# JJanai/back2future

Hardware: AMD Instinct MI355X
Metric: frame-triplets/sec at 3x1024x1920 (higher is better)
Workload: dtype f32; 1 GPU; BASELINE.json configs[4] per-GPU share: batch=16 synthetic 3x1024x1920 triplets per GPU, random-init pwc.lua weights (Ours-Hard shape), outputs flow + occ + est[3]; batch_per_gpu=16, global_batch=16, height=1024, width=1920, parallelism=dp1: independent triplets per rank, one RCCL weight broadcast at init, hip_graph=True

## Files before the change

### back2future_amd/csrc/b2f_api.hip

```cpp
#include "b2f_ctx.h"

#include <cctype>
#include <cmath>
#include <cstdio>
#include <cstdlib>

using namespace b2f;

static thread_local std::string g_err;
namespace b2f {
int api_fail(const std::string &m)
{
    g_err = m;
    return 1;
}
const std::string &api_error() { return g_err; }

ConvSeg cp8_seg(const float *ptr, int C, size_t hw)
{
    ConvSeg sgm;
    sgm.ptr = ptr;
    sgm.img_stride = (long)(hw * (size_t)((C + 7) / 8 * 8));
    sgm.chunk_stride = (long)(hw * 8);
    sgm.pix_stride = 8;
    sgm.nchunks = 0;
    return sgm;
}
}
static int fail(const std::string &m) { return api_fail(m); }

namespace {

int prof_id(b2f_ctx *c, const char *name)
{
    for (size_t i = 0; i < c->prof_names.size(); ++i)
        if (c->prof_names[i] == name) return (int)i;
    c->prof_names.push_back(name);
    c->prof_ms.push_back(0.0);
    c->prof_n.push_back(0);
    return (int)c->prof_names.size() - 1;
}

hipEvent_t get_event(b2f_ctx *c)
{
    if (!c->ev_pool.empty()) {
        hipEvent_t e = c->ev_pool.back();
        c->ev_pool.pop_back();
        return e;
    }
    hipEvent_t e = nullptr;
    (void)hipEventCreate(&e);
    return e;
}

struct Scope {
    b2f_ctx *c;
    hipStream_t s;
    ProfEvent pe;
    bool on;
    Scope(b2f_ctx *c_, hipStream_t s_, const char *name, bool capturing) : c(c_), s(s_), on(c_->profile && !capturing)
    {
        if (on) {
            pe.name = prof_id(c, name);
            pe.a = get_event(c);
            pe.b = get_event(c);
            (void)hipEventRecord(pe.a, s);
        }
    }
    ~Scope()
    {
        if (on) {
            (void)hipEventRecord(pe.b, s);
            c->prof_pending.push_back(pe);
        }
    }
};

int prof_collect(b2f_ctx *c)
{
    for (ProfEvent &pe : c->prof_pending) {
        HIPCHK(hipEventSynchronize(pe.b));
        float ms = 0.f;
        HIPCHK(hipEventElapsedTime(&ms, pe.a, pe.b));
        c->prof_ms[pe.name] += ms;
        c->prof_n[pe.name] += 1;
        c->ev_pool.push_back(pe.a);
        c->ev_pool.push_back(pe.b);
    }
    c->prof_pending.clear();
    return 0;
}

int find_conv(const b2f_ctx *c, int kind, int level, int idx);

bool use_wino()
{
    static const bool on = !(getenv("B2F_WINO") && atoi(getenv("B2F_WINO")) == 0);
    return on;
}

struct KernelRow {
    const char *tag[2];
    const char *cls[2];
    void (*tiles)(int co, int *nt, int *nblk);
    size_t (*w_floats)(int chunks, int co, int nt, int nblk);
    bool bias;
    void (*pack)(const float *w, const float *b, int co, int ci, const int *cin_map, int chunks, int nt, int nblk, float *wpk, float *bpk);
    hipError_t (*launch)(const ConvLaunch &, hipStream_t);
};
#define TL [](int co, int *nt, int *nblk)
#define WF [](int chunks, int co, int nt, int nblk) -> size_t
#define PK [](const float *w, const float *b, int co, int ci, const int *m, int chunks, int nt, int nblk, float *wpk, float *bpk)
const KernelRow kKernels[K_COUNT] = {
    {{"D1", "D2"}, {"conv3x3_s1_nt%d", "conv3x3_s2_nt%d"}, conv_choose_tiles, WF { return conv_wpk_floats(chunks, nt, nblk); }, true,
     PK { conv_pack_weights(w, b, co, ci, m, chunks, nt, nblk, wpk, bpk); }, launch_conv3x3},
    {{"N2", "N2"}, {"conv3x3_narrow2", "conv3x3_narrow2"}, TL { *nt = 1; *nblk = 1; }, WF { return narrow2_wpk_floats(chunks); }, true,
     PK { narrow2_pack_weights(w, b, ci, m, chunks, wpk, bpk); }, launch_conv_narrow2},
    {{"W2", "W2"}, {"conv3x3_wino_nt%d", "conv3x3_wino_nt%d"}, wino_choose_tiles, WF { return wino_wpk_floats(chunks, nt, nblk); }, true,
     PK { wino_pack_weights(w, b, co, ci, m, chunks, nt, nblk, wpk, bpk); }, launch_conv3x3_wino},
    {{"C16", "C16"}, {"conv3x3_c16_%d", "conv3x3_c16_%d"}, TL { *nt = 1; *nblk = 1; }, WF { return c16_wpk_floats(); }, true,
     PK { c16_pack_weights(w, b, ci, m, wpk, bpk); }, launch_conv3x3_c16},
    {{"S16", "S16"}, {"conv3x3_s2x16_%d", "conv3x3_s2x16_%d"}, TL { *nt = 1; *nblk = 1; }, WF { return c16s2_wpk_floats(); }, true,
     PK { c16s2_pack_weights(w, b, ci, m, wpk, bpk); }, launch_conv3x3_c16s2},
    {{"W4", "W4"}, {"conv3x3_wino4_nt%d", "conv3x3_wino4_nt%d"}, TL { *nt = 2; *nblk = wino4_nblk(co); }, WF { return wino4_wpk_floats(chunks, nblk); }, true,
     PK { wino4_pack_weights(w, b, co, ci, m, chunks, nblk, wpk, bpk); }, launch_conv3x3_wino4},
    {{"E1", "E2"}, {"conv3x3_s1_bf16_%d", "conv3x3_s2_bf16_%d"}, TL { *nt = 2; *nblk = convb_nblk(co); }, WF { return convb_wpk_floats(chunks, co); }, true,
     PK { convb_pack_weights(w, b, co, ci, m, chunks, wpk, bpk); }, launch_conv3x3_bf6},
    {{"L2", "L2"}, {"conv3x3_s2b_%d", "conv3x3_s2b_%d"}, TL { *nt = 1; *nblk = s2b_ntiles(co); }, WF { return s2b_wpk_floats(chunks, co); }, true,
     PK { s2b_pack_weights(w, b, co, ci, m, chunks, wpk, bpk); }, launch_conv3x3_s2b},
    {{"V1", "V1"}, {"conv3x3_w1b_%d", "conv3x3_w1b_%d"}, TL { *nt = 2; *nblk = w1b_nblk(co); }, WF { return w1b_wpk_floats(chunks, co); }, true,
     PK { w1b_pack_weights(w, b, co, ci, m, chunks, wpk, bpk); },
     [](const ConvLaunch &L, hipStream_t s) {
         const hipError_t e = launch_conv3x3_w1b(L, s);
         return e == hipSuccess && L.w1b_nblk < w1b_nblk(L.cout) ? launch_conv3x3_wino4_rem(L, s) : e;
     }},
    {{"W6", "W6"}, {"conv3x3_wino6_nt%d", "conv3x3_wino6_nt%d"}, TL { *nt = 2; *nblk = wino6_nblk(co); }, WF { return wino6_wpk_floats(chunks, co); }, true,
     PK { wino6_pack_weights(w, b, co, ci, m, chunks, wpk, bpk); }, launch_conv3x3_wino6},
#if B2F_EXPERIMENTS
    {{nullptr, nullptr}, {nullptr, nullptr}, TL { *nt = 2; *nblk = wino4_nblk(co); }, WF { return wino4s_wpk_floats(chunks, nblk); }, false,
     PK { wino4s_pack_weights(w, co, ci, m, chunks, nblk, wpk); }, nullptr},
    {{nullptr, nullptr}, {nullptr, nullptr}, TL { *nt = 2; *nblk = wino4_nblk(co); }, WF { return wino2s_wpk_floats(chunks, nblk); }, false,
     PK { wino2s_pack_weights(w, co, ci, m, chunks, nblk, wpk); }, nullptr},
#endif
};
#undef TL
#undef WF
#undef PK

ConvKernel base_kernel(int ci, int co, bool stride1, bool two_segments)
{
    static const int min4 = getenv("B2F_WINO4_MIN_COUT") ? atoi(getenv("B2F_WINO4_MIN_COUT")) : 32;
    static const int min2 = getenv("B2F_WINO_MIN_COUT") ? atoi(getenv("B2F_WINO_MIN_COUT")) : 16;
    if (!use_wino()) return K_DIRECT;
    if (ci == 16 && co == (stride1 ? 16 : 32)) return stride1 ? K_C16 : K_C16S2;
    if (!stride1) return K_DIRECT;
    if (co == 2) return two_segments ? K_DIRECT : K_NARROW2;
    if (co < min2) return K_DIRECT;
    return (min4 > 0 && co >= min4 && co % 4 == 0) ? K_WINO4 : K_WINO2;
}

bool packs(const PackedConv &p, ConvKernel k, bool stride1, const KernelOpts &o)
{
    const bool w4 = p.base == K_WINO4;
    switch (k) {
    case K_BF6: return (p.base == K_DIRECT || (w4 && o.bf16_conv >= 2)) && (p.cout & 3) == 0;
    case K_S2B: return p.base == K_DIRECT && !stride1 && (p.cout & 31) == 0 && p.cout <= 256;
    case K_WINO2: return w4 || p.base == K_WINO2;
    case K_W1B: return w4 && o.wino1d;
    case K_WINO6: return w4 && o.wino6;
#if B2F_EXPERIMENTS
    case K_WINO4S: return w4 && (o.wino4_split || o.wino4_hybrid);
    case K_WINO2S: return w4 && o.wino2_split;
#endif
    default: return k == p.base;
    }
}

void place_packings(PackedConv &p, bool stride1, const KernelOpts &o, size_t *total)
{
    for (int k = 0; k < K_COUNT; ++k) {
        if (!packs(p, (ConvKernel)k, stride1, o)) continue;
        PackedConv::Packing &q = p.pk[k];
        kKernels[k].tiles(p.cout, &q.nt, &q.nblk);
        q.w_off = *total = (*total + 3) & ~(size_t)3;
        q.b_off = *total += kKernels[k].w_floats(p.nchunks(), p.cout, q.nt, q.nblk);
        if (kKernels[k].bias) *total += (size_t)q.nblk * q.nt * 32;
    }
}

void fill_packings(const PackedConv &p, const float *w, const float *b, int ci, const int *cin_map, float *host)
{
    for (int k = 0; k < K_COUNT; ++k)
        if (p.has((ConvKernel)k))
            kKernels[k].pack(w, b, p.cout, ci, cin_map, p.nchunks(), p.pk[k].nt, p.pk[k].nblk, host + p.pk[k].w_off, host + p.pk[k].b_off);
}

int pack_all(b2f_ctx *c, const float *flat)
{
    const size_t n = c->lay.size();
    c->packed.assign(n, PackedConv());
    size_t total = 0;
    std::vector<std::vector<int>> maps(n);
    for (size_t i = 0; i < n; ++i) {
        const ConvDesc &d = c->lay[i];
        PackedConv &p = c->packed[i];
        p.cout = d.co;
        const bool stride1 = !(d.kind == KIND_FEAT && d.idx == 1 && d.level >= 2);
        p.base = base_kernel(d.ci, d.co, stride1, d.kind != KIND_FEAT && d.idx == 1);
        std::vector<int> &m = maps[i];
        if (d.kind != KIND_FEAT && d.idx == 1 && c->g.shipped()) {
            const int Cl = kFeat[d.level];
            const bool has_feat = d.ci >= kND + Cl;
            const bool has_flow = d.ci == kND + Cl + 2;
            if (has_feat) {
                p.nseg = 2;
                p.chunks[0] = Cl / kCK;
                for (int k = 0; k < Cl; ++k) m.push_back(kND + k);
            } else {
                p.nseg = 1;
            }
            p.chunks[p.nseg - 1] = kCvChunks;
            const int flow_at = (d.kind == KIND_PAST) ? 164 : 162;
            for (int k = 0; k < kCvRec; ++k) {
                int ci = -1;
                if (k < 80) ci = k;
                else if (k < 160) ci = 81 + (k - 80);
                else if (k == 160) ci = 80;
                else if (k == 161) ci = 161;
                else if (has_flow && k >= flow_at && k < flow_at + 2) ci = kND + Cl + (k - flow_at);
                m.push_back(ci);
            }
        } else {
            p.nseg = 1;
            p.chunks[0] = (d.ci + kCK - 1) / kCK;
            for (int k = 0; k < p.chunks[0] * kCK; ++k) m.push_back(k < d.ci ? k : -1);
        }
        place_packings(p, stride1, *c, &total);
    }
    c->first_w_off = total; total += 27 * 16;
    c->first_b_off = total; total += 16;
    std::vector<float> host(total, 0.f);
    const int id_first = find_conv(c, KIND_FEAT, 2, 1);
    if (id_first >= 0 && c->lay[(size_t)id_first].ci == 3 && c->lay[(size_t)id_first].co == 16) {
        const ConvDesc &d = c->lay[(size_t)id_first];
        for (int o = 0; o < 16; ++o) {
            for (int t = 0; t < 27; ++t) host[c->first_w_off + (size_t)t * 16 + o] = flat[d.w_off + (size_t)o * 27 + t];
            host[c->first_b_off + o] = flat[d.b_off + o];
        }
    }
    for (size_t i = 0; i < n; ++i)
        fill_packings(c->packed[i], flat + c->lay[i].w_off, flat + c->lay[i].b_off, c->lay[i].ci, maps[i].data(), host.data());
    if (c->wpk_floats != total) {
        if (c->wpk_dev) HIPCHK(hipFree(c->wpk_dev));
        c->wpk_dev = nullptr;
        HIPCHK(hipMalloc(&c->wpk_dev, total * sizeof(float)));
        c->wpk_floats = total;
    }
    HIPCHK(hipMemcpy(c->wpk_dev, host.data(), total * sizeof(float), hipMemcpyHostToDevice));
    return 0;
}

int find_conv(const b2f_ctx *c, int kind, int level, int idx)
{
    for (size_t i = 0; i < c->lay.size(); ++i)
        if (c->lay[i].kind == kind && c->lay[i].level == level && c->lay[i].idx == idx) return (int)i;
    return -1;
}

struct Plan {
    int B, H, W;
    bool full;
    bool seq;
    int nimg;
    int fo;
    int rec;
    int h[8], w[8];
    size_t img, tmp, cs[8], U[8], UB[8], cv, d[6], fs, bfs, logits, u2, flow_planar, ds[6], total;
};

Plan make_plan(int B, int H, int W, bool full, bool past_flow, bool seq = false)
{
    Plan p;
    p.B = B; p.H = H; p.W = W;
    p.full = full;
    p.seq = seq;
    p.nimg = seq ? B + 2 : 3 * B;
    p.fo = seq ? 1 : B;
    p.rec = kCvRec;
    for (int l = 1; l <= 7; ++l) { p.h[l] = H >> (l - 1); p.w[l] = W >> (l - 1); }
    size_t off = 0;
    auto take = [&](size_t n) { size_t o = off; off += (n + 63) & ~(size_t)63; return o; };
    p.img = full ? take((size_t)3 * B * H * W * kImgC) : 0;
    p.tmp = take((size_t)p.nimg * p.h[2] * p.w[2] * kFeat[2]);
    for (int l = 2; l <= 7; ++l) p.cs[l] = take((size_t)p.nimg * p.h[l] * p.w[l] * kFeat[l]);
    for (int l = 3; l <= 6; ++l) p.U[l] = take((size_t)B * p.h[l] * p.w[l] * 2);
    for (int l = 3; l <= 6; ++l) p.UB[l] = (full && past_flow) ? take((size_t)B * p.h[l] * p.w[l] * 2) : 0;
    p.cv = take((size_t)B * p.h[3] * p.w[3] * p.rec + 64);
    const size_t px3 = (size_t)B * p.h[3] * p.w[3];
    for (int i = 1; i <= 5; ++i) p.d[i] = take(px3 * kDec[i]);
    p.fs = take(px3 * 8);
    p.bfs = take(px3 * 8);
    p.logits = take(px3 * 8);
    p.u2 = take(px3 * 4 * 2);
    p.flow_planar = take((size_t)B * 2 * H * W);
    for (int k = 2; k <= 5; ++k) p.ds[k] = full ? take((size_t)2 * B * (H >> (k - 1)) * (W >> (k - 1)) * kImgC) : 0;
    p.total = off;
    return p;
}

}
void b2f::drop_gen_out(b2f_ctx *c)
{
    for (float *p : c->gen_out)
        if (p) (void)hipFree(p);
    c->gen_out.clear();
    c->genB = c->genH = c->genW = 0;
}
void b2f::drop_graphs(b2f_ctx *c)
{
    for (auto &g : c->graphs)
        if (g.second) (void)hipGraphExecDestroy(g.second);
    c->graphs.clear();
}
namespace {

int ensure_workspace_floats(b2f_ctx *c, size_t total)
{
    if (total > c->arena_floats) {
        if (c->arena) {
            HIPCHK(hipDeviceSynchronize());
            HIPCHK(hipFree(c->arena));
            c->arena = nullptr;
            c->arena_floats = 0;
            drop_graphs(c);
        }
        HIPCHK(hipMalloc(&c->arena, total * sizeof(float)));
        HIPCHK(hipMemset(c->arena, 0, total * sizeof(float)));
        HIPCHK(hipDeviceSynchronize());
        c->arena_floats = total;
    }
    return 0;
}
int ensure_workspace(b2f_ctx *c, const Plan &p) { return ensure_workspace_floats(c, p.total); }

struct KernelChoice {
    ConvKernel kernel;
    bool f2x2;
    int nsplit;
    int w1b_blocks;
};

KernelChoice choose_kernel(const PackedConv &p, const KernelOpts &o, int cur_batch, const ConvLaunch &L)
{
    const int H = L.H, W = L.W;
    bool alt = false, split = false;
    if (p.base == K_WINO4) {
        const PackedConv::Packing &p2 = p.pk[K_WINO2];
        const bool per_launch = o.adaptive_kernels > 0 || (o.adaptive_kernels < 0 && cur_batch == 1);
        if (!per_launch) {
            alt = H * W < o.wino4_min_pixels;
            split = alt && p2.nt == 2 && H * W <= o.wino_split_pixels;
        } else {
            const long tiles2 = (long)L.nimg * ((H + 7) / 8) * ((W + 15) / 16);
            const long b4 = (long)L.nimg * ((H + 15) / 16) * ((W + 31) / 32) * p.pk[K_WINO4].nblk;
            const long b2 = tiles2 * p2.nblk, b2s = tiles2 * ((p.cout + 31) / 32);
            const long t4 = 60 * ((b4 + 255) / 256);
            const long t2 = b2 <= 256 ? 20 : 40 * ((b2 + 511) / 512);
            const long t2s = p2.nt != 2 ? t2 : b2s <= 256 ? 13 : 26 * ((b2s + 511) / 512);
            alt = std::min(t2, t2s) < t4;
            split = alt && t2s < t2;
        }
    }
    const ConvKernel mode = alt ? K_WINO2 : p.base;
    KernelChoice ch = {mode, alt, split ? 1 : 0, 0};
    const bool big4 = mode == K_WINO4 && L.stride == 1;
    if (p.has(K_BF6) && ((mode == K_DIRECT && o.bf16_conv) || (big4 && H * W >= o.bf16_conv_min_pixels && ((o.bf16_conv == 2 && p.cout <= 32) || o.bf16_conv >= 3))) &&
        convb_supported(L))
        ch.kernel = K_BF6;
    if (mode == K_DIRECT && L.stride == 2 && o.bf16_conv && o.s2_loader && p.has(K_S2B) && (o.s2_loader >= 2 || p.nchunks() >= 8) && s2b_supported(L)) {
        ch.kernel = K_S2B;
        ch.nsplit = o.s2_tile_groups ? 0 : -1;
    }
    if (big4 && ch.kernel == K_WINO4) {
        const int blocks = o.wino1d >= 2 ? w1b_nblk(p.cout) : p.cout / 64 + (p.cout % 64 > 32 ? 1 : 0);
        if (o.wino1d && p.has(K_W1B) && blocks > 0 && w1b_supported(L)) {
            ch.kernel = K_W1B;
            ch.w1b_blocks = blocks;
        } else if (o.wino6 && p.has(K_WINO6) && H * W >= o.wino6_min_pixels && wino6_supported(L)) {
            ch.kernel = K_WINO6;
        }
    }
    return ch;
}

int launch_layer(b2f_ctx *c, hipStream_t s, bool prof, const PackedConv &p, const float *wpk, const KernelOpts &o, int cur_batch, ConvLaunch &L)
{
    for (int i = 0; i < p.nseg; ++i) L.seg[i].nchunks = p.chunks[i];
    if (p.nseg == 1) L.seg[1] = L.seg[0], L.seg[1].nchunks = 0;
    L.nseg = p.nseg;
    L.cout = p.cout;
    L.Ho = (L.H + 2 - 3) / L.stride + 1;
    L.Wo = (L.W + 2 - 3) / L.stride + 1;
    L.tiles_per_block = o.s2_tiles_per_block;
    L.w4_persist = o.wino4_persistent;
    L.w8 = o.wino8;
    L.bf16_direct = o.bf16_direct;
    auto weights = [&](ConvKernel k) { return p.has(k) ? wpk + p.pk[k].w_off : nullptr; };
    auto bias = [&](ConvKernel k) { return p.has(k) ? wpk + p.pk[k].b_off : nullptr; };
    L.wpk_bf6 = weights(K_BF6); L.bias_bf6 = bias(K_BF6);
    L.wpk_s2b = weights(K_S2B); L.bias_s2b = bias(K_S2B);
    L.wpk_w1b = weights(K_W1B); L.bias_w1b = bias(K_W1B);
    L.wpk_w6 = weights(K_WINO6); L.bias_w6 = bias(K_WINO6);
    const KernelChoice ch = choose_kernel(p, o, cur_batch, L);
    const PackedConv::Packing &q = p.pk[ch.f2x2 ? K_WINO2 : p.base];
    L.wpk = wpk + q.w_off;
    L.bias = wpk + q.b_off;
    L.nt = q.nt;
    L.nblk = q.nblk;
    L.nsplit = ch.nsplit;
    L.w1b_nblk = ch.w1b_blocks;
#if B2F_EXPERIMENTS
    if (!ch.f2x2) { L.wpk_split = weights(K_WINO4S); L.wpk_split2 = weights(K_WINO2S); }
    L.w4_hybrid = o.wino4_hybrid;
#endif
    const KernelRow &k = kKernels[ch.kernel];
    char name[48];
    if (c->profile_layers)
        snprintf(name, sizeof name, "conv%s_%dto%d_%dx%d", (B2F_EXPERIMENTS && ch.kernel == K_C16 && o.bf16_direct) ? "B16" : k.tag[L.stride - 1],
                 p.nchunks() * 8, p.cout, L.H, L.W);
    else
        snprintf(name, sizeof name, k.cls[L.stride - 1], L.nt);
    Scope sc(c, s, name, !prof);
    HIPCHK(k.launch(L, s));
    return 0;
}

int run_conv(b2f_ctx *c, hipStream_t s, bool cap, int conv_id, const ConvSeg *segs, int nimg, int H, int W,
             int stride, int leaky, float *out)
{
    const PackedConv &p = c->packed[conv_id];
    ConvLaunch L{};
    for (int i = 0; i < p.nseg; ++i) L.seg[i] = segs[i];
    L.out = out;
    L.H = H; L.W = W; L.stride = stride;
    const size_t hwo = (size_t)((H + 2 - 3) / stride + 1) * ((W + 2 - 3) / stride + 1);
    L.out_img_stride = (long)(hwo * ((p.cout + 7) / 8 * 8));
    L.out_chunk_stride = (long)(hwo * 8);
    L.out_pix_stride = 8;
    L.nimg = nimg;
    L.leaky = leaky;
    return launch_layer(c, s, !cap, p, c->wpk_dev, *c, c->cur_batch, L);
}

int run_decoder(b2f_ctx *c, hipStream_t s, bool cap, const Plan &P, int kind, int l, float *out2)
{
    const size_t *dbuf = P.d;
    float *A = c->arena;
    const int h = P.h[l], w = P.w[l], B = P.B;
    const size_t hw = (size_t)h * w;
    const int Cl = kFeat[l];
    const int id1 = find_conv(c, kind, l, 1);
    if (id1 < 0) return fail("decoder not present in this model");
    ConvSeg segs[2];
    const ConvSeg seg_ref = cp8_seg(A + P.cs[l] + (size_t)P.fo * hw * Cl, Cl, hw);
    const ConvSeg seg_cv = cp8_seg(A + P.cv, kCvRec, hw);
    if (c->packed[id1].nseg == 2) { segs[0] = seg_ref; segs[1] = seg_cv; }
    else { segs[0] = seg_cv; segs[1] = seg_cv; }
    CHK(run_conv(c, s, cap, id1, segs, B, h, w, 1, 1, A + dbuf[1]));
    for (int i = 2; i <= 6; ++i) {
        const ConvSeg in = cp8_seg(A + dbuf[i - 1], kDec[i - 1], hw);
        float *o = (i == 6) ? out2 : A + dbuf[i];
        CHK(run_conv(c, s, cap, find_conv(c, kind, l, i), &in, B, h, w, 1, i < 6, o));
    }
    return 0;
}

struct Outs {
    float *flow = nullptr, *occ = nullptr, *est3 = nullptr;
    float *t_ufs[8] = {nullptr}, *t_ubfs[8] = {nullptr}, *t_occ[8] = {nullptr}, *t_iw1[8] = {nullptr}, *t_iw3[8] = {nullptr};
};

int forward_impl(b2f_ctx *c, hipStream_t s, bool cap, const void *dev_in, int in_kind, const Plan &P, const Outs &O)
{
    c->cur_batch = c->req_batch > 0 ? c->req_batch : P.B;
    float *A = c->arena;
    const int B = P.B;
    const bool full = P.full, past = c->past_flow && full;
    const int unit = in_kind == B2F_IN_UNIT;
    if (full) {
        Scope sc(c, s, "pack_input", cap);
        HIPCHK(launch_pack_input((const float *)dev_in, unit, B, P.H, P.W, A + P.img, s));
    }
    const int head_id1 = find_conv(c, KIND_FEAT, 2, 2), head_id2 = find_conv(c, KIND_FEAT, 3, 1);
    const bool head_fused = c->bf16_direct >= 2 && P.h[2] >= 4 && P.w[2] >= 4 && head_id1 >= 0 && head_id2 >= 0 &&
                            c->packed[(size_t)head_id1].base == K_C16 && c->packed[(size_t)head_id2].base == K_C16S2;
    for (int l = 2; l <= 7; ++l) {
        const int hi = P.h[l - 1], wi = P.w[l - 1], ho = P.h[l], wo = P.w[l];
        const int Ci = (l == 2) ? kImgC : kFeat[l - 1], Co = kFeat[l];
        if (l == 2 && P.seq) {
            Scope sc(c, s, "conv_first_seq", cap);
            HIPCHK(launch_conv_first_seq(dev_in, in_kind, P.nimg, P.H, P.W, c->wpk_dev + c->first_w_off, c->wpk_dev + c->first_b_off,
                                         A + P.tmp, s));
        } else if (l == 2) {
            Scope sc(c, s, "conv_first", cap);
            HIPCHK(launch_conv_first((const float *)dev_in, unit, B, P.H, P.W, c->wpk_dev + c->first_w_off,
                                     c->wpk_dev + c->first_b_off, A + P.tmp, s));
        } else if (l == 3 && head_fused) {
            const ConvSeg in2f = cp8_seg(A + P.cs[2], Co, (size_t)ho * wo);
            CHK(run_conv(c, s, cap, find_conv(c, KIND_FEAT, l, 2), &in2f, P.nimg, ho, wo, 1, 1, A + P.cs[l]));
            continue;
        } else {
            const ConvSeg in1 = cp8_seg(A + P.cs[l - 1], Ci, (size_t)hi * wi);
            CHK(run_conv(c, s, cap, find_conv(c, KIND_FEAT, l, 1), &in1, P.nimg, hi, wi, 2, 1, A + P.tmp));
        }
        if (l == 2 && head_fused) {
            const PackedConv::Packing &p1 = c->packed[(size_t)head_id1].pk[K_C16], &p2 = c->packed[(size_t)head_id2].pk[K_C16S2];
            HeadLaunch hl;
            hl.in = A + P.tmp; hl.in_img_stride = (long)((size_t)ho * wo * 16); hl.in_chunk_stride = (long)((size_t)ho * wo * 8); hl.in_pix_stride = 8;
            hl.H1 = ho; hl.W1 = wo;
            hl.w1 = c->wpk_dev + p1.w_off; hl.b1 = c->wpk_dev + p1.b_off; hl.w2 = c->wpk_dev + p2.w_off; hl.b2 = c->wpk_dev + p2.b_off;
            hl.out = A + P.cs[2];
            hl.Ho = P.h[3]; hl.Wo = P.w[3]; hl.nimg = P.nimg;
            hl.out_img_stride = (long)((size_t)hl.Ho * hl.Wo * 32); hl.out_chunk_stride = (long)((size_t)hl.Ho * hl.Wo * 8); hl.out_pix_stride = 8;
            char hname[48];
            snprintf(hname, sizeof hname, c->profile_layers ? "convH16_16to32_%dx%d" : "conv_head16_bf16", ho, wo);
            Scope sc(c, s, hname, cap);
            HIPCHK(launch_conv_head16(hl, s));
            continue;
        }
        const ConvSeg in2 = cp8_seg(A + P.tmp, Co, (size_t)ho * wo);
        CHK(run_conv(c, s, cap, find_conv(c, KIND_FEAT, l, 2), &in2, P.nimg, ho, wo, 1, 1, A + P.cs[l]));
    }
    if (full) {
        Scope sc(c, s, "avgpool2", cap);
        const size_t img_f = (size_t)B * P.H * P.W * kImgC;
        for (int f = 0; f < 2; ++f) {
            const float *src = A + P.img + (size_t)(f == 0 ? 0 : 2) * img_f;
            for (int k = 2; k <= 5; ++k) {
                const int hk = P.H >> (k - 2), wk = P.W >> (k - 2);
                float *dst = A + P.ds[k] + (size_t)f * B * (hk / 2) * (wk / 2) * kImgC;
                HIPCHK(launch_avgpool2_nhwc(src, B, hk, wk, kImgC, dst, s));
                src = dst;
            }
        }
    }
    for (int l = 7; l >= 3; --l) {
        const int h = P.h[l], w = P.w[l], Cl = kFeat[l];
        const size_t hw = (size_t)h * w;
        CorrLaunch cl;
        cl.ref = A + P.cs[l] + (size_t)P.fo * hw * Cl;
        cl.nbr_fut = A + P.cs[l] + (size_t)2 * P.fo * hw * Cl;
        cl.nbr_past = A + P.cs[l];
        cl.img_stride = (long)(hw * Cl);
        cl.chunk_stride = (long)(hw * 8);
        cl.pix_stride = 8;
        cl.flow = (l < 7) ? A + P.U[l] : nullptr;
        cl.flow_b = (l < 7 && past) ? A + P.UB[l] : nullptr;
        cl.k = (float)(20.0 / std::pow(2.0, l - 1));
        cl.out = A + P.cv;
        cl.out_img_stride = (long)(hw * kCvRec);
        cl.out_chunk_stride = (long)(hw * 8);
        cl.out_pix_stride = 8;
        cl.B = B; cl.C = Cl; cl.h = h; cl.w = w;
        cl.variant = c->corr_variant;
        cl.ablate = c->corr_ablate;
        {
            char cname[48];
            snprintf(cname, sizeof cname, c->profile_layers ? "warp_costvol_%dx%d" : "warp_costvol", h, w);
            Scope sc(c, s, cname, cap);
            HIPCHK(launch_warp_costvol(cl, s));
        }
        float *occ_out = full ? O.t_occ[l] : (l == 3 ? O.occ : nullptr);
        float *occ_out2 = (!full && l == 3 && c->past_flow) ? O.est3 : nullptr;
        if (occ_out || occ_out2) {
            CHK(run_decoder(c, s, cap, P, KIND_OCC, l, A + P.logits));
            {
                Scope sc(c, s, "softmax_nearest4", cap);
                if (occ_out) HIPCHK(launch_softmax_nearest4_planar(A + P.logits, 8, B, h, w, occ_out, s));
                if (occ_out2) HIPCHK(launch_softmax_nearest4_planar(A + P.logits, 8, B, h, w, occ_out2, s));
            }
        }
        CHK(run_decoder(c, s, cap, P, KIND_FLOW, l, A + P.fs));
        if (past) CHK(run_decoder(c, s, cap, P, KIND_PAST, l, A + P.bfs));
        float *skip_f = full ? O.t_ufs[l] : (l == 3 ? (O.flow ? O.flow : A + P.flow_planar) : nullptr);
        {
            Scope sc(c, s, "upsample_flow2x", cap);
            float *u = (l > 3) ? A + P.U[l - 1] : A + P.u2;
            HIPCHK(launch_upsample_flow2x(A + P.fs, 8, B, h, w, u, s));
            if (skip_f) HIPCHK(launch_upsample_flow2x_planar(u, 2, B, 2 * h, 2 * w, skip_f, s));
            if (past) {
                float *ub = (l > 3) ? A + P.UB[l - 1] : A + P.d[1];
                HIPCHK(launch_upsample_flow2x(A + P.bfs, 8, B, h, w, ub, s));
                if (O.t_ubfs[l]) HIPCHK(launch_upsample_flow2x_planar(ub, 2, B, 2 * h, 2 * w, O.t_ubfs[l], s));
            }
        }
        if (full) {
            Scope sc(c, s, "warp_image", cap);
            const int k = l - 2;
            const int hk = 4 * h, wk = 4 * w;
            const size_t img_f = (size_t)B * hk * wk * kImgC;
            const float *im1 = (k == 1) ? A + P.img : A + P.ds[k];
            const float *im3 = (k == 1) ? A + P.img + 2 * img_f : A + P.ds[k] + img_f;
            const float kk = (float)(20.0 / std::pow(2.0, l - 3));
            const float *fl1 = (past && O.t_ubfs[l]) ? O.t_ubfs[l] : O.t_ufs[l];
            if (O.t_iw1[l]) HIPCHK(launch_warp_image_planar(im1, fl1, -kk, B, hk, wk, O.t_iw1[l], s));
            if (O.t_iw3[l]) HIPCHK(launch_warp_image_planar(im3, O.t_ufs[l], kk, B, hk, wk, O.t_iw3[l], s));
        }
    }
    if (!full && O.est3 && !c->past_flow && P.seq) {
        Scope sc(c, s, "warp_image_seq", cap);
        HIPCHK(launch_warp_input_seq(dev_in, in_kind, O.flow ? O.flow : A + P.flow_planar, -20.0f, B, P.H, P.W, O.est3, s));
    } else if (!full && O.est3 && !c->past_flow) {
        Scope sc(c, s, "warp_image", cap);
        HIPCHK(launch_warp_input_planar((const float *)dev_in, unit, 0, O.flow ? O.flow : A + P.flow_planar, -20.0f, B, P.H, P.W,
                                        O.est3, s));
    }
    return 0;
}

}
int b2f::find_conv_id(const b2f_ctx *c, int kind, int level, int idx) { return find_conv(c, kind, level, idx); }
int b2f::run_conv_layer(b2f_ctx *c, hipStream_t s, bool cap, int conv_id, const ConvSeg *segs, int nimg, int H, int W, int stride,
                        int leaky, float *out)
{
    if (conv_id < 0) return fail("b2f: layer not present in this model");
    return run_conv(c, s, cap, conv_id, segs, nimg, H, W, stride, leaky, out);
}
int b2f::ensure_arena(b2f_ctx *c, size_t floats) { return ensure_workspace_floats(c, floats); }
int b2f::check_shape(int B, int H, int W)
{
    if (B <= 0 || H <= 0 || W <= 0) return fail("b2f: non-positive shape");
    if (H % 64 || W % 64) return fail("b2f: H and W must be multiples of 64 (7 pyramid levels, back2future.lua:54-67)");
    return 0;
}
namespace {

bool parse_random(const char *name, bool *past, unsigned long long *seed, float *gain)
{
    if (strncmp(name, "random:", 7) != 0) return false;
    std::string s(name + 7);
    std::vector<std::string> parts;
    size_t pos = 0;
    while (true) {
        size_t q = s.find(':', pos);
        parts.push_back(s.substr(pos, q == std::string::npos ? q : q - pos));
        if (q == std::string::npos) break;
        pos = q + 1;
    }
    if (parts[0] == "hard") *past = false;
    else if (parts[0] == "soft") *past = true;
    else return false;
    *seed = 2;
    *gain = 1.f;
    if (parts.size() > 1 && !parts[1].empty()) *seed = strtoull(parts[1].c_str(), nullptr, 10);
    if (parts.size() > 2 && !parts[2].empty()) *gain = strtof(parts[2].c_str(), nullptr);
    return true;
}

bool ends_with(const std::string &s, const char *suf)
{
    const size_t n = strlen(suf);
    return s.size() >= n && s.compare(s.size() - n, n, suf) == 0;
}

int install_weights(b2f_ctx *c, const float *flat, long long n, bool past)
{
    GraphOpts g = c->g;
    g.past_flow = past;
    if (n != param_count(g)) return fail("b2f: weight count does not match the architecture");
    HIPCHK(hipDeviceSynchronize());
    drop_graphs(c);
    drop_gen_out(c);
    if (c->w_dev && (c->nparams != n)) { HIPCHK(hipFree(c->w_dev)); c->w_dev = nullptr; }
    c->past_flow = past;
    c->g = g;
    c->nparams = n;
    long long t = 0;
    c->lay = weight_layout(g, &t);
    if (!c->w_dev) HIPCHK(hipMalloc(&c->w_dev, (size_t)n * sizeof(float)));
    HIPCHK(hipMemcpy(c->w_dev, flat, (size_t)n * sizeof(float), hipMemcpyHostToDevice));
    return pack_all(c, flat);
}

enum {
    OPT_ENV = 1,
    OPT_SYNC = 2,
    OPT_EXP_ONLY = 4,
};
struct OptRow {
    const char *name;
    int b2f_ctx::*member;
    int flags;
    int repack;
};
const OptRow kOptions[] = {
    {"use_graph", &b2f_ctx::use_graph, OPT_ENV, 0},
    {"host_graph", &b2f_ctx::host_graph, OPT_ENV, 0},
    {"profile", &b2f_ctx::profile, OPT_ENV, 0},
    {"profile_layers", &b2f_ctx::profile_layers, OPT_ENV, 0},
    {"corr_variant", &b2f_ctx::corr_variant, OPT_ENV | OPT_SYNC, 0},
    {"corr_ablate", &b2f_ctx::corr_ablate, OPT_ENV | OPT_SYNC, 0},
    {"bf16_direct", &b2f_ctx::bf16_direct, OPT_ENV | OPT_SYNC, 0},
    {"bf16_conv", &b2f_ctx::bf16_conv, OPT_ENV | OPT_SYNC, 1},
    {"bf16_conv_min_pixels", &b2f_ctx::bf16_conv_min_pixels, OPT_SYNC, 0},
    {"wino1d", &b2f_ctx::wino1d, OPT_ENV | OPT_SYNC, 2},
    {"wino6", &b2f_ctx::wino6, OPT_ENV | OPT_SYNC, 3},
    {"wino6_min_pixels", &b2f_ctx::wino6_min_pixels, OPT_ENV | OPT_SYNC, 0},
    {"wino2_split", &b2f_ctx::wino2_split, OPT_ENV | OPT_SYNC | OPT_EXP_ONLY, 4},
    {"wino4_split", &b2f_ctx::wino4_split, OPT_ENV | OPT_SYNC | OPT_EXP_ONLY, 5},
    {"wino4_hybrid", &b2f_ctx::wino4_hybrid, OPT_ENV | OPT_SYNC | OPT_EXP_ONLY, 5},
    {"s2_tiles_per_block", &b2f_ctx::s2_tiles_per_block, OPT_ENV | OPT_SYNC, 0},
    {"wino4_persistent", &b2f_ctx::wino4_persistent, OPT_ENV | OPT_SYNC, 0},
    {"s2_loader", &b2f_ctx::s2_loader, OPT_ENV | OPT_SYNC, 0},
    {"s2_tile_groups", &b2f_ctx::s2_tile_groups, OPT_ENV | OPT_SYNC, 0},
    {"wino_split_pixels", &b2f_ctx::wino_split_pixels, OPT_ENV | OPT_SYNC, 0},
    {"wino8", &b2f_ctx::wino8, OPT_ENV | OPT_SYNC, 0},
    {"wino4_min_pixels", &b2f_ctx::wino4_min_pixels, OPT_ENV | OPT_SYNC, 0},
    {"adaptive_kernels", &b2f_ctx::adaptive_kernels, OPT_ENV | OPT_SYNC, 0},
    {"op_wino_split", &b2f_ctx::op_wino_split, OPT_ENV, 0},
    {"host_subbatch_pixels", nullptr, OPT_ENV, 0},
    {"host_threads", &b2f_ctx::host_threads, OPT_ENV, 0},
    {"host_u8", &b2f_ctx::host_u8, OPT_ENV, 0},
    {"host_ramp", &b2f_ctx::host_ramp, OPT_ENV, 0},
    {"debug_fail_next", &b2f_ctx::debug_fail_next, 0, 0},
};

const OptRow *find_option(const char *key)
{
    for (const OptRow &r : kOptions)
        if (!strcmp(key, r.name)) return &r;
    return nullptr;
}

bool reads_packing(const b2f_ctx *c, int group)
{
    for (const OptRow &r : kOptions)
        if (r.repack == group && (r.member == &b2f_ctx::bf16_conv ? c->*r.member >= 2 : c->*r.member != 0)) return true;
    return false;
}

const char *experiment_value(const OptRow &r, int value)
{
    if (B2F_EXPERIMENTS) return nullptr;
    if (r.member == &b2f_ctx::corr_variant && (value == 2 || value == 4 || value == 6 || value == 8))
        return "b2f_set_option: corr_variant 2 / 4 / 6 / 8 are experiment kernels: build with `python -m back2future_amd.build --experiments`";
    if (r.member == &b2f_ctx::bf16_direct && value == 1)
        return "b2f_set_option: bf16_direct = 1 (the 16 -> 16 layer alone on the bf16 pipe) is an experiment: build with `python -m back2future_amd.build --experiments`";
    return nullptr;
}

}

extern "C" {

const char *b2f_last_error(void) { return g_err.c_str(); }
int b2f_version(void) { return 1001; }

long long b2f_param_count(int past_flow) { return param_count(past_flow != 0); }

int b2f_random_weights(unsigned long long seed, int past_flow, float gain, float *out, long long n) try
{
    if (!out || n != param_count(past_flow != 0)) return fail("b2f_random_weights: bad buffer size");
    random_weights(seed, past_flow != 0, gain, out);
    return 0;
}
B2F_CATCH("b2f_random_weights")

int b2f_load_t7(const char *path, float *out, long long cap, long long *n, int *past_flow) try
{
    std::vector<float> flat;
    bool past = false;
    std::string err;
    if (!path) return fail("b2f_load_t7: null path");
    if (!load_t7(path, flat, past, err)) return fail("b2f_load_t7: " + err);
    if (n) *n = (long long)flat.size();
    if (past_flow) *past_flow = past ? 1 : 0;
    if (out) {
        if (cap < (long long)flat.size()) return fail("b2f_load_t7: output buffer too small");
        memcpy(out, flat.data(), flat.size() * sizeof(float));
    }
    return 0;
}
B2F_CATCH("b2f_load_t7")

int b2f_load_t7_ex(const char *path, const char *graph_opts, float *out, long long cap, long long *n, char *opts_out, int opts_cap) try
{
    if (!path) return fail("b2f_load_t7_ex: null path");
    GraphOpts g;
    std::string err;
    if (!parse_graph_opts(graph_opts, g, err)) return fail("b2f_load_t7_ex: " + err);
    std::vector<float> flat;
    if (!load_t7_ex(path, g, !(graph_opts && *graph_opts), flat, err)) return fail("b2f_load_t7_ex: " + err);
    if (n) *n = (long long)flat.size();
    if (opts_out && opts_cap > 0) {
        const std::string t = graph_opts_string(g);
        if ((int)t.size() + 1 > opts_cap) return fail("b2f_load_t7_ex: option buffer too small");
        memcpy(opts_out, t.c_str(), t.size() + 1);
    }
    if (out) {
        if (cap < (long long)flat.size()) return fail("b2f_load_t7_ex: output buffer too small");
        memcpy(out, flat.data(), flat.size() * sizeof(float));
    }
    return 0;
}
B2F_CATCH("b2f_load_t7_ex")

int b2f_init(const char *name_or_path, int device, b2f_ctx **out) { return b2f_init_ex(name_or_path, device, nullptr, out); }

int b2f_init_ex(const char *name_or_path, int device, const char *graph_opts, b2f_ctx **out) try
{
    if (!out) return fail("b2f_init: null out");
    *out = nullptr;
    GraphOpts g;
    {
        std::string err;
        if (!parse_graph_opts(graph_opts, g, err)) return fail("b2f_init: " + err);
    }
    int ndev = 0;
    if (hipGetDeviceCount(&ndev) != hipSuccess || ndev <= 0)
        return fail("b2f_init: no HIP device available (this library has no CPU fallback)");
    if (device < 0 || device >= ndev) return fail("b2f_init: bad device ordinal");
    HIPCHK(hipSetDevice(device));
    const char *name = name_or_path ? name_or_path : "Ours-Soft-ft-KITTI";
    std::vector<float> flat;
    bool past = false;
    unsigned long long seed = 2;
    float gain = 1.f;
    if (parse_random(name, &past, &seed, &gain)) {
        g.past_flow = past;
        flat.resize((size_t)param_count(g));
        random_weights(seed, g, gain, flat.data());
    } else {
        std::string path = name;
        if (path == "Ours-Hard") path = "models/RoamingImages_H.t7";
        else if (path == "Ours-Soft-ft-KITTI") path = "models/RoamingImages_H_KITTI_S.t7";
        else if (path == "Ours-Soft-ft-Sintel") path = "models/RoamingImages_H_Sintel_S.t7";
        if (ends_with(path, ".t7")) {
            std::string err;
            if (!load_t7_ex(path, g, !(graph_opts && *graph_opts), flat, err)) return fail("b2f_init: " + err);
            past = g.past_flow;
        } else if (ends_with(path, ".b2fw")) {
            FILE *f = fopen(path.c_str(), "rb");
            if (!f) return fail("b2f_init: cannot open " + path);
            fseek(f, 0, SEEK_END);
            const long sz = ftell(f);
            fseek(f, 0, SEEK_SET);
            flat.resize((size_t)sz / 4);
            const size_t rd = fread(flat.data(), 4, flat.size(), f);
            fclose(f);
            if (rd != flat.size()) return fail("b2f_init: short read on " + path);
            GraphOpts gp = g, gn = g;
            gp.past_flow = true; gn.past_flow = false;
            if ((long long)flat.size() == param_count(gp)) past = true;
            else if ((long long)flat.size() == param_count(gn)) past = false;
            else return fail("b2f_init: " + path + " does not hold a parameter set of this graph (with or without past-flow decoders)");
        } else {
            return fail(std::string("b2f_init: unknown model '") + name + "'");
        }
    }
    b2f_ctx *c = new b2f_ctx();
    c->device = device;
    c->g = g;
    {
        auto env_int = [](const std::string &k, long long dflt) {
            const char *v = getenv(k.c_str());
            if (!v) return dflt;
            char *end = nullptr;
            const long long x = strtoll(v, &end, 10);
            return end == v ? 1ll : x;
        };
        if (!use_wino()) { c->bf16_conv = 0; c->bf16_direct = 0; }
// ... 562 lines not shown
```

### back2future_amd/csrc/b2f_ctx.h

```cpp
#pragma once
#include "../../include/b2f.h"

#include <algorithm>
#include <atomic>
#include <condition_variable>
#include <cstring>
#include <exception>
#include <map>
#include <memory>
#include <mutex>
#include <string>
#include <thread>
#include <tuple>
#include <vector>

#include "b2f_host.h"
#include "b2f_internal.h"

namespace b2f {

int api_fail(const std::string &m);
const std::string &api_error();


enum ConvKernel {
    K_DIRECT = 0,
    K_NARROW2,
    K_WINO2,
    K_C16,
    K_C16S2,
    K_WINO4,
    K_BF6,
    K_S2B,
    K_W1B,
    K_WINO6,
#if B2F_EXPERIMENTS
    K_WINO4S,
    K_WINO2S,
#endif
    K_COUNT
};

struct PackedConv {
    int nseg = 1;
    int chunks[2] = {0, 0};
    int cout = 0;
    ConvKernel base = K_DIRECT;
    struct Packing {
        size_t w_off = 0, b_off = 0;
        int nt = 0, nblk = 0;
    } pk[K_COUNT];
    bool has(ConvKernel k) const { return pk[k].nblk != 0; }
    int nchunks() const { return chunks[0] + (nseg > 1 ? chunks[1] : 0); }
};

struct KernelOpts {
    int wino8 = 1;
    int wino_split_pixels = 512;
    int wino4_min_pixels = 4096;
    int adaptive_kernels = -1;
    int bf16_direct = 2;
    int bf16_conv_min_pixels = 65536;
    int bf16_conv = 1;
    int wino2_split = 0;
    int wino4_hybrid = 0;
    int wino4_split = 0;
    int wino6 = 1;
    int wino6_min_pixels = 16384;
    int wino1d = 0;
    int s2_tile_groups = 1;
    int s2_loader = 1;
    int wino4_persistent = 1;
    int s2_tiles_per_block = 0;
};

struct ProfEvent {
    int name;
    hipEvent_t a, b;
};

struct GraphKey {
    const void *in;
    float *flow, *occ, *est3;
    int kind, B, H, W;
    int rule;
    int seq;
    bool operator<(const GraphKey &o) const
    {
        return std::tie(in, flow, occ, est3, kind, B, H, W, rule, seq) < std::tie(o.in, o.flow, o.occ, o.est3, o.kind, o.B, o.H, o.W, o.rule, o.seq);
    }
};

struct HostSlot {
    char *dev = nullptr;
    size_t dev_bytes = 0;
    char *pin = nullptr;
    size_t pin_bytes = 0;
    unsigned char *d_u8 = nullptr;
    float *d_up = nullptr, *d_tmp = nullptr, *d_in = nullptr, *d_flow = nullptr, *d_est3 = nullptr;
    float *d_flow32 = nullptr;
    float *d_occ = nullptr;
    float *d_prob = nullptr;
    unsigned char *d_fo = nullptr, *d_bo = nullptr;
    unsigned char *d_rgb = nullptr;
    double *d_max = nullptr;
    unsigned char *h_u8 = nullptr;
    float *h_in = nullptr, *h_flow32 = nullptr, *h_prob = nullptr;
    unsigned char *h_fo = nullptr, *h_bo = nullptr, *h_rgb = nullptr;
    double *h_max = nullptr;
    hipEvent_t ev_in = nullptr, ev_comp = nullptr, ev_out = nullptr;
};

struct FlowOutputs {
    double *flow64 = nullptr;
    float *flow32 = nullptr, *occ_prob = nullptr;
    unsigned char *fwd_occ = nullptr, *bwd_occ = nullptr;
    unsigned char *rgb = nullptr;
    double *rgb_max = nullptr;
    double max_norm = 0.0;
    int rgb_layout = B2F_RGB_PLANAR;
    bool pictures = false;
    bool f32() const { return flow64 == nullptr; }
    FlowOutputs from_triplet(size_t b, size_t hw0) const
    {
        auto at = [](auto *p, size_t off) { return p ? p + off : p; };
        return {at(flow64, b * 2 * hw0), at(flow32, b * 2 * hw0), at(occ_prob, b * 2 * hw0), at(fwd_occ, b * hw0), at(bwd_occ, b * hw0),
                at(rgb, b * 3 * hw0), at(rgb_max, b), max_norm, rgb_layout, pictures};
    }
};

inline FlowOutputs rgb_outputs(unsigned char *rgb, double *max_used, double max_norm, int layout, float *flow, unsigned char *fwd_occ,
                               unsigned char *bwd_occ)
{
    return {nullptr, flow, nullptr, fwd_occ, bwd_occ, rgb, max_used, max_norm, layout, true};
}

struct FlowRequest {
    int n = 0;
    bool seq = false;
    int in_kind = B2F_IN_UNIT;
    const void *im1 = nullptr, *im2 = nullptr, *im3 = nullptr;
    int H0 = 0, W0 = 0;
    FlowOutputs o;
    int req = 0;
    const char *who = "";
};

inline FlowRequest batch_request(const char *who, int n, int in_kind, const void *im1, const void *im2, const void *im3, int H0, int W0,
                                 const FlowOutputs &o)
{
    return {n, false, in_kind, im1, im2, im3, H0, W0, o, 0, who};
}

inline FlowRequest sequence_request(const char *who, int T, int in_kind, const void *frames, int H0, int W0, const FlowOutputs &o)
{
    return {T >= 3 ? T - 2 : 0, true, in_kind, frames, nullptr, nullptr, H0, W0, o, 0, who};
}

struct DevWork {
    char *dev = nullptr;
    size_t bytes = 0;
};

enum { JOB_COPY = 0, JOB_F32_TO_F64 = 1, JOB_PACK_U8 = 2 };
struct CopyJob {
    void *dst;
    const void *src;
    size_t bytes;
    int kind = JOB_COPY;
    double scale = 1.0;
    std::atomic<int> *inexact = nullptr;
};

inline bool pack_u8_piece(unsigned char *d, const float *s, size_t n)
{
    uint32_t bad = 0;
    for (size_t i = 0; i < n; ++i) {
        const float v = s[i];
        int k = (int)(v * 255.0f + 0.5f);
        k = k < 0 ? 0 : (k > 255 ? 255 : k);
        const float r = (float)k / 255.0f;
        uint32_t vb, rb;
        memcpy(&vb, &v, 4);
        memcpy(&rb, &r, 4);
        bad |= vb ^ rb;
        d[i] = (unsigned char)k;
    }
    return bad == 0;
}

inline void run_piece(const CopyJob &j)
{
    if (j.kind == JOB_COPY) {
        memcpy(j.dst, j.src, j.bytes);
    } else if (j.kind == JOB_F32_TO_F64) {
        const float *s = (const float *)j.src;
        double *d = (double *)j.dst;
        const double sc = j.scale;
        for (size_t i = 0, n = j.bytes / 4; i < n; ++i) d[i] = (double)s[i] * sc;
    } else {
        if (!pack_u8_piece((unsigned char *)j.dst, (const float *)j.src, j.bytes / 4)) j.inexact->store(1, std::memory_order_relaxed);
    }
}

class CopyPool {
public:
    explicit CopyPool(int workers)
    {
        for (int i = 0; i < workers; ++i) th_.emplace_back([this] { worker(); });
    }
    ~CopyPool()
    {
        {
            std::lock_guard<std::mutex> l(m_);
            stop_ = true;
        }
        cv_.notify_all();
        for (std::thread &t : th_) t.join();
    }
    int workers() const { return (int)th_.size(); }
    void run(const std::vector<CopyJob> &jobs)
    {
        constexpr size_t kPiece = 1 << 20;
        std::vector<CopyJob> pieces;
        size_t bytes = 0;
// ... 128 lines not shown
```

Measured before the change: 833.7 triplets/s.

## Merge first conv of occ/flow/past decoders into one wide launch

Packs the weights of the first decoder conv for the occlusion, flow and past-flow decoders contiguously, so one Winograd launch computes all of them over the shared cost-volume input. The output goes into a wider interleaved buffer, and each decoder's remaining convs read its slice through an adjusted image stride. This is meant to avoid reading the large cost volume several times and to cut the number of launches. In exchange it enlarges the d[1] buffer, makes the packing layout more complex, and falls back to separate launches when layouts or sizes don't allow a merge.

```diff
diff --git a/back2future_amd/csrc/b2f_api.hip b/back2future_amd/csrc/b2f_api.hip
--- a/back2future_amd/csrc/b2f_api.hip
+++ b/back2future_amd/csrc/b2f_api.hip
@@ -107,6 +107,7 @@
     bool bias;
     void (*pack)(const float *w, const float *b, int co, int ci, const int *cin_map, int chunks, int nt, int nblk, float *wpk, float *bpk);
     hipError_t (*launch)(const ConvLaunch &, hipStream_t);
+    bool nblock_major = false;
 };
 #define TL [](int co, int *nt, int *nblk)
 #define WF [](int chunks, int co, int nt, int nblk) -> size_t
@@ -117,13 +118,13 @@
     {{"N2", "N2"}, {"conv3x3_narrow2", "conv3x3_narrow2"}, TL { *nt = 1; *nblk = 1; }, WF { return narrow2_wpk_floats(chunks); }, true,
      PK { narrow2_pack_weights(w, b, ci, m, chunks, wpk, bpk); }, launch_conv_narrow2},
     {{"W2", "W2"}, {"conv3x3_wino_nt%d", "conv3x3_wino_nt%d"}, wino_choose_tiles, WF { return wino_wpk_floats(chunks, nt, nblk); }, true,
-     PK { wino_pack_weights(w, b, co, ci, m, chunks, nt, nblk, wpk, bpk); }, launch_conv3x3_wino},
+     PK { wino_pack_weights(w, b, co, ci, m, chunks, nt, nblk, wpk, bpk); }, launch_conv3x3_wino, true},
     {{"C16", "C16"}, {"conv3x3_c16_%d", "conv3x3_c16_%d"}, TL { *nt = 1; *nblk = 1; }, WF { return c16_wpk_floats(); }, true,
      PK { c16_pack_weights(w, b, ci, m, wpk, bpk); }, launch_conv3x3_c16},
     {{"S16", "S16"}, {"conv3x3_s2x16_%d", "conv3x3_s2x16_%d"}, TL { *nt = 1; *nblk = 1; }, WF { return c16s2_wpk_floats(); }, true,
      PK { c16s2_pack_weights(w, b, ci, m, wpk, bpk); }, launch_conv3x3_c16s2},
     {{"W4", "W4"}, {"conv3x3_wino4_nt%d", "conv3x3_wino4_nt%d"}, TL { *nt = 2; *nblk = wino4_nblk(co); }, WF { return wino4_wpk_floats(chunks, nblk); }, true,
-     PK { wino4_pack_weights(w, b, co, ci, m, chunks, nblk, wpk, bpk); }, launch_conv3x3_wino4},
+     PK { wino4_pack_weights(w, b, co, ci, m, chunks, nblk, wpk, bpk); }, launch_conv3x3_wino4, true},
     {{"E1", "E2"}, {"conv3x3_s1_bf16_%d", "conv3x3_s2_bf16_%d"}, TL { *nt = 2; *nblk = convb_nblk(co); }, WF { return convb_wpk_floats(chunks, co); }, true,
      PK { convb_pack_weights(w, b, co, ci, m, chunks, wpk, bpk); }, launch_conv3x3_bf6},
     {{"L2", "L2"}, {"conv3x3_s2b_%d", "conv3x3_s2b_%d"}, TL { *nt = 1; *nblk = s2b_ntiles(co); }, WF { return s2b_wpk_floats(chunks, co); }, true,
@@ -135,7 +136,7 @@
          return e == hipSuccess && L.w1b_nblk < w1b_nblk(L.cout) ? launch_conv3x3_wino4_rem(L, s) : e;
      }},
     {{"W6", "W6"}, {"conv3x3_wino6_nt%d", "conv3x3_wino6_nt%d"}, TL { *nt = 2; *nblk = wino6_nblk(co); }, WF { return wino6_wpk_floats(chunks, co); }, true,
-     PK { wino6_pack_weights(w, b, co, ci, m, chunks, wpk, bpk); }, launch_conv3x3_wino6},
+     PK { wino6_pack_weights(w, b, co, ci, m, chunks, wpk, bpk); }, launch_conv3x3_wino6, true},
 #if B2F_EXPERIMENTS
     {{nullptr, nullptr}, {nullptr, nullptr}, TL { *nt = 2; *nblk = wino4_nblk(co); }, WF { return wino4s_wpk_floats(chunks, nblk); }, false,
      PK { wino4s_pack_weights(w, co, ci, m, chunks, nblk, wpk); }, nullptr},
@@ -185,6 +186,36 @@
         q.w_off = *total = (*total + 3) & ~(size_t)3;
         q.b_off = *total += kKernels[k].w_floats(p.nchunks(), p.cout, q.nt, q.nblk);
         if (kKernels[k].bias) *total += (size_t)q.nblk * q.nt * 32;
+    }
+}
+
+void place_side_by_side(PackedConv *const *ps, int n, bool stride1, const KernelOpts &o, size_t *total)
+{
+    for (int k = 0; k < K_COUNT; ++k) {
+        if (!packs(*ps[0], (ConvKernel)k, stride1, o)) continue;
+        size_t wf = 0;
+        int nt = 0, nblk = 0;
+        kKernels[k].tiles(ps[0]->cout, &nt, &nblk);
+        if (kKernels[k].nblock_major) wf = kKernels[k].w_floats(ps[0]->nchunks(), ps[0]->cout, nt, nblk);
+        const bool side = kKernels[k].nblock_major && kKernels[k].bias && nt == 2 && (wf & 3) == 0;
+        for (int pass = 0; pass < (side ? 2 : 1); ++pass)
+            for (int j = 0; j < n; ++j) {
+                PackedConv::Packing &q = ps[j]->pk[k];
+                if (!side) {
+                    kKernels[k].tiles(ps[j]->cout, &q.nt, &q.nblk);
+                    q.w_off = *total = (*total + 3) & ~(size_t)3;
+                    q.b_off = *total += kKernels[k].w_floats(ps[j]->nchunks(), ps[j]->cout, q.nt, q.nblk);
+                    if (kKernels[k].bias) *total += (size_t)q.nblk * q.nt * 32;
+                } else if (pass == 0) {
+                    q.nt = nt; q.nblk = nblk;
+                    if (j == 0) *total = (*total + 3) & ~(size_t)3;
+                    q.w_off = *total;
+                    *total += wf;
+                } else {
+                    q.b_off = *total;
+                    *total += (size_t)nblk * nt * 32;
+                }
+            }
     }
 }
 
@@ -235,7 +266,26 @@
             p.chunks[0] = (d.ci + kCK - 1) / kCK;
             for (int k = 0; k < p.chunks[0] * kCK; ++k) m.push_back(k < d.ci ? k : -1);
         }
-        place_packings(p, stride1, *c, &total);
+    }
+    std::vector<char> placed(n, 0);
+    for (size_t i = 0; i < n; ++i) {
+        if (placed[i]) continue;
+        const ConvDesc &d = c->lay[i];
+        PackedConv &p = c->packed[i];
+        const bool stride1 = !(d.kind == KIND_FEAT && d.idx == 1 && d.level >= 2);
+        std::vector<PackedConv *> grp(1, &p);
+        if (d.kind != KIND_FEAT && d.idx == 1 && c->g.shipped() && p.cout % 64 == 0)
+            for (size_t j = i + 1; j < n; ++j) {
+                const ConvDesc &e = c->lay[j];
+                const PackedConv &q = c->packed[j];
+                if (e.kind != KIND_FEAT && e.idx == 1 && e.level == d.level && q.cout == p.cout && q.base == p.base && q.nseg == p.nseg &&
+                    q.chunks[0] == p.chunks[0] && q.chunks[1] == p.chunks[1]) {
+                    grp.push_back(&c->packed[j]);
+                    placed[j] = 1;
+                }
+            }
+        if (grp.size() > 1) place_side_by_side(grp.data(), (int)grp.size(), stride1, *c, &total);
+        else place_packings(p, stride1, *c, &total);
     }
     c->first_w_off = total; total += 27 * 16;
     c->first_b_off = total; total += 16;
@@ -297,7 +347,7 @@
     for (int l = 3; l <= 6; ++l) p.UB[l] = (full && past_flow) ? take((size_t)B * p.h[l] * p.w[l] * 2) : 0;
     p.cv = take((size_t)B * p.h[3] * p.w[3] * p.rec + 64);
     const size_t px3 = (size_t)B * p.h[3] * p.w[3];
-    for (int i = 1; i <= 5; ++i) p.d[i] = take(px3 * kDec[i]);
+    for (int i = 1; i <= 5; ++i) p.d[i] = take(px3 * kDec[i] * (i == 2 && full && past_flow ? 2 : 1));
     p.fs = take(px3 * 8);
     p.bfs = take(px3 * 8);
     p.logits = take(px3 * 8);
@@ -393,7 +443,9 @@
     return ch;
 }
 
-int launch_layer(b2f_ctx *c, hipStream_t s, bool prof, const PackedConv &p, const float *wpk, const KernelOpts &o, int cur_batch, ConvLaunch &L)
+constexpr int kCannotMerge = -1;
+int launch_layer(b2f_ctx *c, hipStream_t s, bool prof, const PackedConv &p, const float *wpk, const KernelOpts &o, int cur_batch, ConvLaunch &L,
+                 const PackedConv *const *more = nullptr, int nmore = 0)
 {
     for (int i = 0; i < p.nseg; ++i) L.seg[i].nchunks = p.chunks[i];
     if (p.nseg == 1) L.seg[1] = L.seg[0], L.seg[1].nchunks = 0;
@@ -424,6 +476,23 @@
     L.w4_hybrid = o.wino4_hybrid;
 #endif
     const KernelRow &k = kKernels[ch.kernel];
+    if (nmore > 0) {
+        const int all = (1 + nmore) * p.cout;
+        if (!k.nblock_major || (o.merge_dec1 > 1 && all > o.merge_dec1)) return kCannotMerge;
+        const PackedConv::Packing *at = &p.pk[ch.kernel];
+        if (at->nt != 2 || p.cout != at->nblk * 64) return kCannotMerge;
+        for (int j = 0; j < nmore; ++j) {
+            const PackedConv::Packing &nx = more[j]->pk[ch.kernel];
+            if (more[j]->cout != p.cout || nx.nblk != at->nblk || nx.nt != at->nt || nx.w_off != at->w_off + k.w_floats(p.nchunks(), p.cout, at->nt, at->nblk) ||
+                nx.b_off != at->b_off + (size_t)at->nblk * 64)
+                return kCannotMerge;
+            at = &nx;
+        }
+        L.cout = all;
+        L.nblk *= 1 + nmore;
+        if (ch.kernel == K_WINO6 ? !wino6_supported(L) : (double)(all / 8) * (double)L.out_chunk_stride * 4.0 + (double)L.Ho * L.Wo * L.out_pix_stride * 4.0 >= 2147483648.0)
+            return kCannotMerge;
+    }
     char name[48];
     if (c->profile_layers)
         snprintf(name, sizeof name, "conv%s_%dto%d_%dx%d", (B2F_EXPERIMENTS && ch.kernel == K_C16 && o.bf16_direct) ? "B16" : k.tag[L.stride - 1],
@@ -436,7 +505,7 @@
 }
 
 int run_conv(b2f_ctx *c, hipStream_t s, bool cap, int conv_id, const ConvSeg *segs, int nimg, int H, int W,
-             int stride, int leaky, float *out)
+             int stride, int leaky, float *out, int out_channels = 0, const int *more_ids = nullptr, int nmore = 0)
 {
     const PackedConv &p = c->packed[conv_id];
     ConvLaunch L{};
@@ -444,12 +513,14 @@
     L.out = out;
     L.H = H; L.W = W; L.stride = stride;
     const size_t hwo = (size_t)((H + 2 - 3) / stride + 1) * ((W + 2 - 3) / stride + 1);
-    L.out_img_stride = (long)(hwo * ((p.cout + 7) / 8 * 8));
+    L.out_img_stride = (long)(hwo * (out_channels > 0 ? out_channels : (p.cout + 7) / 8 * 8));
     L.out_chunk_stride = (long)(hwo * 8);
     L.out_pix_stride = 8;
     L.nimg = nimg;
     L.leaky = leaky;
-    return launch_layer(c, s, !cap, p, c->wpk_dev, *c, c->cur_batch, L);
+    const PackedConv *more[2] = {nullptr, nullptr};
+    for (int j = 0; j < nmore && j < 2; ++j) more[j] = &c->packed[more_ids[j]];
+    return launch_layer(c, s, !cap, p, c->wpk_dev, *c, c->cur_batch, L, more, nmore);
 }
 
 int run_decoder(b2f_ctx *c, hipStream_t s, bool cap, const Plan &P, int kind, int l, float *out2)
@@ -472,6 +543,52 @@
         float *o = (i == 6) ? out2 : A + dbuf[i];
         CHK(run_conv(c, s, cap, find_conv(c, kind, l, i), &in, B, h, w, 1, i < 6, o));
     }
+    return 0;
+}
+
+int run_decoders(b2f_ctx *c, hipStream_t s, bool cap, const Plan &P, int l, const int *kinds, float *const *out2, int n)
+{
+    float *A = c->arena;
+    const int h = P.h[l], w = P.w[l], B = P.B;
+    const size_t hw = (size_t)h * w;
+    const int Cl = kFeat[l];
+    int id1[3] = {-1, -1, -1};
+    for (int j = 0; j < n; ++j)
+        if ((id1[j] = find_conv(c, kinds[j], l, 1)) < 0) return fail("decoder not present in this model");
+    bool merge = c->merge_dec1 != 0 && n >= 2 && n <= 3;
+    for (int j = 1; merge && j < n; ++j) {
+        const PackedConv &a = c->packed[id1[0]], &b = c->packed[id1[j]];
+        merge = a.cout == kDec[1] && b.cout == a.cout && b.base == a.base && b.nseg == a.nseg && b.chunks[0] == a.chunks[0] && b.chunks[1] == a.chunks[1];
+    }
+    if (merge) {
+        const int CM = n * kDec[1];
+        ConvSeg segs[2];
+        const ConvSeg seg_cv = cp8_seg(A + P.cv, kCvRec, hw);
+        segs[0] = c->packed[id1[0]].nseg == 2 ? cp8_seg(A + P.cs[l] + (size_t)P.fo * hw * Cl, Cl, hw) : seg_cv;
+        segs[1] = seg_cv;
+        float *M = A + P.d[1], *R = A + P.d[3], *R5 = R + (size_t)B * hw * kDec[4];
+        const int rc = run_conv(c, s, cap, id1[0], segs, B, h, w, 1, 1, M, CM, id1 + 1, n - 1);
+        if (rc != kCannotMerge) {
+            CHK(rc);
+            for (int j = 0; j < n; ++j) {
+                float *Mj = M + (size_t)j * (kDec[1] / 8) * hw * 8;
+                ConvSeg in = cp8_seg(Mj, kDec[1], hw);
+                in.img_stride = (long)(hw * CM);
+                CHK(run_conv(c, s, cap, find_conv(c, kinds[j], l, 2), &in, B, h, w, 1, 1, R));
+                in = cp8_seg(R, kDec[2], hw);
+                CHK(run_conv(c, s, cap, find_conv(c, kinds[j], l, 3), &in, B, h, w, 1, 1, Mj, CM));
+                in = cp8_seg(Mj, kDec[3], hw);
+                in.img_stride = (long)(hw * CM);
+                CHK(run_conv(c, s, cap, find_conv(c, kinds[j], l, 4), &in, B, h, w, 1, 1, R));
+                in = cp8_seg(R, kDec[4], hw);
+                CHK(run_conv(c, s, cap, find_conv(c, kinds[j], l, 5), &in, B, h, w, 1, 1, R5));
+                in = cp8_seg(R5, kDec[5], hw);
+                CHK(run_conv(c, s, cap, find_conv(c, kinds[j], l, 6), &in, B, h, w, 1, 0, out2[j]));
+            }
+            return 0;
+        }
+    }
+    for (int j = 0; j < n; ++j) CHK(run_decoder(c, s, cap, P, kinds[j], l, out2[j]));
     return 0;
 }
 
@@ -572,16 +689,17 @@
         }
         float *occ_out = full ? O.t_occ[l] : (l == 3 ? O.occ : nullptr);
         float *occ_out2 = (!full && l == 3 && c->past_flow) ? O.est3 : nullptr;
+        int kinds[3], nk = 0;
+        float *dec_out[3];
+        if (occ_out || occ_out2) { kinds[nk] = KIND_OCC; dec_out[nk++] = A + P.logits; }
+        kinds[nk] = KIND_FLOW; dec_out[nk++] = A + P.fs;
+        if (past) { kinds[nk] = KIND_PAST; dec_out[nk++] = A + P.bfs; }
+        CHK(run_decoders(c, s, cap, P, l, kinds, dec_out, nk));
         if (occ_out || occ_out2) {
-            CHK(run_decoder(c, s, cap, P, KIND_OCC, l, A + P.logits));
-            {
-                Scope sc(c, s, "softmax_nearest4", cap);
-                if (occ_out) HIPCHK(launch_softmax_nearest4_planar(A + P.logits, 8, B, h, w, occ_out, s));
-                if (occ_out2) HIPCHK(launch_softmax_nearest4_planar(A + P.logits, 8, B, h, w, occ_out2, s));
-            }
-        }
-        CHK(run_decoder(c, s, cap, P, KIND_FLOW, l, A + P.fs));
-        if (past) CHK(run_decoder(c, s, cap, P, KIND_PAST, l, A + P.bfs));
+            Scope sc(c, s, "softmax_nearest4", cap);
+            if (occ_out) HIPCHK(launch_softmax_nearest4_planar(A + P.logits, 8, B, h, w, occ_out, s));
+            if (occ_out2) HIPCHK(launch_softmax_nearest4_planar(A + P.logits, 8, B, h, w, occ_out2, s));
+        }
         float *skip_f = full ? O.t_ufs[l] : (l == 3 ? (O.flow ? O.flow : A + P.flow_planar) : nullptr);
         {
             Scope sc(c, s, "upsample_flow2x", cap);
@@ -717,6 +835,7 @@
     {"wino8", &b2f_ctx::wino8, OPT_ENV | OPT_SYNC, 0},
     {"wino4_min_pixels", &b2f_ctx::wino4_min_pixels, OPT_ENV | OPT_SYNC, 0},
     {"adaptive_kernels", &b2f_ctx::adaptive_kernels, OPT_ENV | OPT_SYNC, 0},
+    {"merge_dec1", &b2f_ctx::merge_dec1, OPT_ENV | OPT_SYNC, 0},
     {"op_wino_split", &b2f_ctx::op_wino_split, OPT_ENV, 0},
     {"host_subbatch_pixels", nullptr, OPT_ENV, 0},
     {"host_threads", &b2f_ctx::host_threads, OPT_ENV, 0},
diff --git a/back2future_amd/csrc/b2f_ctx.h b/back2future_amd/csrc/b2f_ctx.h
--- a/back2future_amd/csrc/b2f_ctx.h
+++ b/back2future_amd/csrc/b2f_ctx.h
@@ -71,6 +71,7 @@
     int s2_tile_groups = 1;
     int s2_loader = 1;
     int wino4_persistent = 1;
+    int merge_dec1 = 1;
     int s2_tiles_per_block = 0;
 };
 
```

New measurement: 834.0 triplets/s (median of 2 runs). About the same (+0.0%).
